# erthward/geonomics

Measured on AMD Instinct MI355X. Metric: individual-timesteps/sec, higher is better.
Workload: dtype u64

## Files before the change

geonomics_amd/_native.py:

```python
import ctypes as C
import os

import numpy as np

_HERE = os.path.dirname(os.path.abspath(__file__))
LIB_PATH = os.environ.get('GNX_LIB') or os.path.join(_HERE, 'libgnxhip.so')

DIST = {'lognormal': 0, 'wald': 1, 'levy': 2}
MATE_UNIFORM, MATE_NEAREST, MATE_INVERSE = 0, 1, 2
SURF_NONE, SURF_MIXTURE, SURF_UNIMODAL = 0, 1, 2
(F_X, F_Y, F_AGE, F_SEX, F_ID, F_E, F_Z, F_FIT, F_GROW, F_GENO) = range(10)
(R_N, R_NPAIRS, R_K, R_D, R_COUNTS) = range(5)
KERNELS = ['move', 'sort', 'permute', 'find_mates', 'pairs', 'offspring',
           'crossover', 'phenotype', 'density', 'death', 'compact', 'crossover_tail']

EXPORTS = [
    'gnx_create', 'gnx_destroy', 'gnx_last_error', 'gnx_words_per_hom', 'gnx_blocks_per_hom',
    'gnx_set_stream', 'gnx_synchronize', 'gnx_upload_rasters',
    'gnx_upload_layer', 'gnx_set_species_params', 'gnx_upload_population',
    'gnx_init_population', 'gnx_set_recomb_paths', 'gnx_set_trait',
    'gnx_set_dominance', 'gnx_set_deleterious', 'gnx_upload_genomes',
    'gnx_assign_genomes', 'gnx_set_z', 'gnx_age', 'gnx_move',
    'gnx_pop_dynamics', 'gnx_pop_dynamics_mate', 'gnx_pop_dynamics_die',
    'gnx_set_z_range', 'gnx_step', 'gnx_counts', 'gnx_step_index',
# ... 371 lines not shown
        cnt = np.zeros(64, np.int64)
        self._chk(self.lib.gnx_tile2_vt_counts(self.h, _ptr(cnt, C.c_int64)))
        return cnt

    def tile2_vt_bases(self, bases):
        b = _arr(bases, np.int64)
        assert b.size == 64
        self._chk(self.lib.gnx_tile2_vt_bases(self.h, _ptr(b, C.c_int64)))

    def step_begin(self, burn):
        self._chk(self.lib.gnx_step_begin(self.h, int(bool(burn))))

    def step_mid(self, burn, with_selection):
        self._chk(self.lib.gnx_step_mid(self.h, int(bool(burn)), int(bool(with_selection))))

    def step_end(self, burn):
        self._chk(self.lib.gnx_step_end(self.h, int(bool(burn))))

    def counts(self):
        n, b, d = C.c_int64(), C.c_int64(), C.c_int64()
        self._chk(self.lib.gnx_counts(self.h, C.byref(n), C.byref(b), C.byref(d)))
        return n.value, b.value, d.value

    def totals(self):
        out = np.zeros(6, np.int64)
        self._chk(self.lib.gnx_totals(self.h, _ptr(out, C.c_int64)))
        return dict(zip(('steps', 'ind_steps', 'births', 'deaths', 'xo_births', 'dd_steps'),
                        (int(v) for v in out)))

    def reset_totals(self):
        self._chk(self.lib.gnx_reset_totals(self.h))

    PATH_COUNTS = ('lazy_mortalities', 'xo_launch_p2', 'xo_flush', 'jobs_lanes_256',
                   'jobs_lanes_512', 'sort_hist_gather', 'gc_with_pending_xo', 'make_dense')

    def path_counts(self):
        out = np.zeros(len(self.PATH_COUNTS), np.int64)
        n = self.lib.gnx_path_counts(self.h, _ptr(out, C.c_int64), len(out))
        assert n == len(out), 'gnx_path_counts: the library has %d counters' % n
        return dict(zip(self.PATH_COUNTS, (int(v) for v in out)))

    def reset_path_counts(self):
        self._chk(self.lib.gnx_reset_path_counts(self.h))

    @property
    def N(self):
        return self.counts()[0]

    @property
    def step_index(self):
        return self.lib.gnx_step_index(self.h)

    @step_index.setter
    def step_index(self, v):
        self._chk(self.lib.gnx_set_step_index(self.h, C.c_int64(int(v))))

    def synchronize(self):
        self._chk(self.lib.gnx_synchronize(self.h))

    def set_defer_crossover(self, on):
        self._chk(self.lib.gnx_set_defer_crossover(self.h, int(bool(on))))

    def set_crossover_overlap(self, mode):
        self._chk(self.lib.gnx_set_crossover_overlap(self.h, int(mode)))

    def debug_halves(self):
        out = np.zeros(6, np.int64)
# ... 1054 lines not shown
```

geonomics_amd/csrc/gnx_api.hip:

```cpp
#include <cmath>
#include <cstdarg>
#include <algorithm>
#include <atomic>
#include <chrono>
#include "gnx_internal.h"
#include "gnx_rng.h"
#include "gnx_compact.h"

static thread_local char g_err[1024] = "";

void gnx_set_error(const char* fmt, ...) {
  va_list ap;
  va_start(ap, fmt);
  vsnprintf(g_err, sizeof(g_err), fmt, ap);
  va_end(ap);
}

extern "C" const char* gnx_last_error(void) { return g_err; }

extern "C" int gnx_words_per_hom(int32_t L) {
  int w = (L + 63) / 64;
  return ((w + 15) / 16) * 16;
}

// ... 289 lines not shown
      }
      h->row_spread = want;
    }
    GNXCHK(dalloc(&h->free_rows, (size_t)h->cfg.cap_rows));
    const size_t halves = (size_t)h->cfg.cap_rows * h->row_spread * 2 * h->NB;
    GNXCHK(dalloc(&h->hmap, halves));
    GNXCHK(dalloc(&h->half_mark, halves));
    GNXCHK(dalloc(&h->half_free, (size_t)h->cfg.cap_rows * 2 * h->NB));
    GNXCHK(dalloc(&h->half_top, 1));
    HIPCHK(hipMalloc(&h->xo_plan, (size_t)cap * 40));
    GNXCHK(dalloc(&h->gc_cnt, (size_t)h->cfg.cap_rows * 2 * h->NB / GNX_CB + 2));
    GNXCHK(dalloc(&h->gc_off, (size_t)h->cfg.cap_rows * 2 * h->NB / GNX_CB + 2));
    HIPCHK(hipMemset(h->half_mark, 0, halves));
    HIPCHK(hipMalloc((void**)&h->xo_jobs_acc, 2 * sizeof(unsigned long long)));
    HIPCHK(hipMemset(h->xo_jobs_acc, 0, 2 * sizeof(unsigned long long)));
    HIPCHK(hipMemset(h->hmap, 0xff, halves * sizeof(int32_t)));
    HIPCHK(hipMemset(h->half_top, 0, sizeof(int32_t)));
    h->alias_xo = gnx_env_int("GNX_XO_ALIAS", 1) != 0;
  }
  for (int k = 0; k < 2; ++k) {
    GNXCHK(dalloc(&h->key[k], cap));
    GNXCHK(dalloc(&h->perm[k], cap));
  }
  GNXCHK(dalloc(&h->mate, cap));
  for (int k = 0; k < 2; ++k) {
    GNXCHK(dalloc(&h->ord[k], cap));
    GNXCHK(dalloc(&h->keyk[k], cap));
    GNXCHK(dalloc(&h->valk[k], cap));
  }
  GNXCHK(dalloc(&h->newslot, cap));
  GNXCHK(dalloc(&h->fill_cnt, 4));
  HIPCHK(hipEventCreateWithFlags(&h->ev_fill, gnx_order_event_flags()));
  HIPCHK(hipEventCreateWithFlags(&h->ev_alive, gnx_order_event_flags()));
  HIPCHK(hipEventCreateWithFlags(&h->ev_perm_rest, gnx_order_event_flags()));
  {
    const size_t nb = std::max(gnx_os_scratch_bytes((size_t)cap, 24),
                               gnx_os_words_used64((size_t)cap, 64) * sizeof(unsigned int)) + 16;
    HIPCHK(hipMalloc(&h->os_scratch, nb));
    HIPCHK(hipMemset(h->os_scratch, 0, nb));
  }
  GNXCHK(dalloc(&h->os_ktmp, cap));
  GNXCHK(dalloc(&h->os_vtmp, cap));
  GNXCHK(dalloc(&h->cell32, cap));
  GNXCHK(dalloc(&h->ord_cnt, cap / GNX_CB + 2));
  GNXCHK(dalloc(&h->ord_off, cap / GNX_CB + 2));
  HIPCHK(hipEventCreateWithFlags(&h->ev_ord, gnx_order_event_flags()));
  HIPCHK(hipStreamCreate(&h->stream3));
  HIPCHK(hipEventCreateWithFlags(&h->ev_compact, gnx_order_event_flags()));
  h->ord_mode = gnx_env_int("GNX_ORD_SORT", 1) != 0;
  GNXCHK(dalloc(&h->tag, cap));
  HIPCHK(hipMalloc(&h->cand, (size_t)cap * 16));
  GNXCHK(dalloc(&h->flag, cap + 1));
  GNXCHK(dalloc(&h->flag2, cap + 1));
  GNXCHK(dalloc(&h->scan, cap + 1));
  GNXCHK(dalloc(&h->pairs, cap * 2));
  GNXCHK(dalloc(&h->nbirths, cap + 1));
  GNXCHK(dalloc(&h->boff, cap + 1));
  GNXCHK(dalloc(&h->off_pair, cap));
  GNXCHK(dalloc(&h->off_parent, cap * 2));
  GNXCHK(dalloc(&h->off_keys, cap * 2));
  GNXCHK(dalloc(&h->off_start, cap * 2));
  GNXCHK(dalloc(&h->keep_in, cap));
  GNXCHK(dalloc(&h->inj_a, cap * GNX_DISP_ATTEMPTS));
  GNXCHK(dalloc(&h->inj_b, cap * GNX_DISP_ATTEMPTS));
  GNXCHK(dalloc(&h->mid_x, cap));
  GNXCHK(dalloc(&h->mid_y, cap));
// ... 89 lines not shown
                  h->delet_loci, h->delet_s, h->cell_start, h->tag, h->cand, h->sort64_tmp, h->key64[0], h->key64[1], h->pairs2,
                  h->pair_goff, h->st_rec, h->st_z, h->st_geno, h->st_slots, h->req_pid, h->req_k, h->req_key, h->req_start, h->req_px, h->req_py,
                  h->req_count, h->sort_tmp, h->scan_tmp, h->mate,
                  h->flag, h->flag2, h->scan, h->pairs, h->nbirths, h->boff, h->off_pair,
                  h->off_parent, h->off_keys, h->off_start, h->keep_in, h->inj_a, h->inj_b,
                  h->mid_x, h->mid_y, h->p_death, h->d_cell, h->dead_in, h->nmax_bits, h->red,
                  h->sel_loci, h->path_sel, h->lat.areas, h->lat.cprime, h->spl_N.c, h->spl_P.c, h->bin_partials, h->nodes,
                  h->K_over, h->blk_cnt, h->blk_off, h->cnt_dev, h->tickets, h->nmax2, h->fb[0], h->gp_rec, h->gp_z, h->gp_slots, h->tile_counts, h->rq_sorted, h->rq_k, h->gam_out, h->gam_slot, h->chk,
                  h->lin_tab, h->lin_bt};
  for (void* p : ptrs) (void)hipFree(p);
  for (int t = 0; t < GNX_MAX_TRAITS; ++t) {
    (void)hipFree(h->traits[t].loci);
    (void)hipFree(h->traits[t].alpha);
    (void)hipFree(h->traits[t].phi_rast);
  }
  (void)hipHostFree(h->h_pin);
  if (h->h_route_pin) (void)hipHostFree(h->h_route_pin);
  (void)hipFree(h->gh_rec);
  (void)hipFree(h->route_cnt);
  if (h->h_stage) (void)hipHostFree(h->h_stage);
  for (int k = 0; k < GNX_K_COUNT; ++k) timers_resolve(h, k);
  for (hipEvent_t e : h->ev_free) (void)hipEventDestroy(e);
  if (h->own_stream) (void)hipStreamDestroy(h->stream);
  if (h->stream2) (void)hipStreamDestroy(h->stream2);
  h->stream2 = nullptr;
  if (h->stream3) {
    (void)hipStreamSynchronize(h->stream3);
    (void)hipStreamDestroy(h->stream3);
  }
  if (h->ev_ord) (void)hipEventDestroy(h->ev_ord);
  if (h->ev_compact) (void)hipEventDestroy(h->ev_compact);
  if (h->ev_fill) (void)hipEventDestroy(h->ev_fill);
  if (h->ev_alive) (void)hipEventDestroy(h->ev_alive);
  if (h->ev_perm_rest) (void)hipEventDestroy(h->ev_perm_rest);
  if (h->ev_pairs) (void)hipEventDestroy(h->ev_pairs);
  if (h->ev_latP) (void)hipEventDestroy(h->ev_latP);
  if (h->ev_perm) (void)hipEventDestroy(h->ev_perm);
  if (h->ev_binsN) (void)hipEventDestroy(h->ev_binsN);
  delete h;
}

extern "C" int gnx_set_stream(gnx_state* h, void* hip_stream) {
  GNXCHK(gnx_xo_join(h));
  HIPCHK(hipStreamSynchronize(h->stream));
  if (h->stream2) HIPCHK(hipStreamSynchronize(h->stream2));
  if (h->own_stream) (void)hipStreamDestroy(h->stream);
  if (h->stream2) (void)hipStreamDestroy(h->stream2);
  h->stream2 = nullptr;
  h->stream = (hipStream_t)hip_stream;
  h->own_stream = false;
  return 0;
}

extern "C" int gnx_synchronize(gnx_state* h) {
  GNXCHK(gnx_xo_launch_pending(h));
  if (h->stream3) HIPCHK(hipStreamSynchronize(h->stream3));
  HIPCHK(hipStreamSynchronize(h->stream));
  if (h->stream2) HIPCHK(hipStreamSynchronize(h->stream2));
  return 0;
}

extern "C" int gnx_upload_rasters(gnx_state* h, const float* rasts) {
  size_t n = (size_t)h->cfg.n_layers * h->cfg.W * h->cfg.H;
  HIPCHK(hipMemcpyAsync(h->rast, rasts, n * sizeof(float), hipMemcpyHostToDevice, h->stream));
  HIPCHK(hipStreamSynchronize(h->stream));
  return 0;
// ... 497 lines not shown
  return 0;
}

extern "C" int gnx_pop_dynamics(gnx_state* h, int32_t burn, int32_t with_selection) {
  GNXCHK(gnx_pop_dynamics_mate(h, burn));
  return gnx_pop_dynamics_die(h, burn, with_selection);
}

struct GnxStepTimer {
  std::chrono::steady_clock::time_point t0 = std::chrono::steady_clock::now();
  bool count;
  explicit GnxStepTimer(bool c) : count(c) {}
  ~GnxStepTimer() {
    if (gnx_host_times()) {
      g_host_step_s += std::chrono::duration<double>(std::chrono::steady_clock::now() - t0).count();
      if (count) ++g_host_steps;
    }
  }
};

extern "C" int gnx_step_begin(gnx_state* h, int32_t burn) {
  GNXCHK(need_params(h));
  GNXCHK(check_recomb_ready(h, burn != 0));
  GnxStepTimer timer(true);
  if (h->mort_wait || h->pairs_wait) {
    gnx_set_error("gnx_step_begin: the previous step of this handle was not finished (gnx_step_end)");
    return 1;
  }
  h->tot[0] += 1;
  h->tot[1] += h->N - h->n_ghost;
  h->last_xo_births = 0;
  h->step_burn = burn != 0;
  h->tile2_mode = false;
  if (h->sp.move) {
    h->move_writes_keys = h->sp.mating_radius >= 0;
    int rc = gnx_l_move(h, true, nullptr, nullptr, nullptr, nullptr, true);
    h->move_writes_keys = false;
    GNXCHK(rc);
  } else {
    GNXCHK(gnx_l_age(h));
  }
  GNXCHK(gnx_l_sort_by_cell(h, true));
  int rc_pairs = gnx_l_find_pairs_enqueue(h, nullptr, true);
  GNXCHK(gnx_wait_permute_rest(h));
  return rc_pairs;
}

extern "C" int gnx_step_mid(gnx_state* h, int32_t burn, int32_t with_selection) {
  GnxStepTimer timer(false);
  int64_t P = 0, B = 0;
  GNXCHK(gnx_l_find_pairs_finish(h, &P));
  if (P > 0 && !h->spl_P.valid)
    GNXCHK(gnx_l_density(h, P, h->mid_x, h->mid_y, &h->spl_P, nullptr));
  GNXCHK(gnx_l_mate(h, burn != 0, false, 0, &B));
  h->last_births = B;
  GNXCHK(gnx_l_density_N(h));
  GNXCHK(gnx_l_death_probs(h, with_selection != 0 && !burn));
  return gnx_l_mortality_enqueue(h, nullptr);
}

extern "C" int gnx_step_end(gnx_state* h, int32_t burn) {
  GnxStepTimer timer(false);
  int64_t D = 0;
  GNXCHK(gnx_l_mortality_finish(h, &D));
  h->last_deaths = D;
  h->step += 1;
  h->tot[2] += h->last_births;
// ... 527 lines not shown
```

geonomics_amd/csrc/gnx_dd.hip:

```cpp
#include <atomic>
#include <chrono>
#include <map>
#include <string>
#include "gnx_internal.h"

bool gnx_fused_bins(const gnx_state* h);

namespace {
using GraphMap = std::map<uint32_t, hipGraphExec_t>;

struct DDExtra {
  GraphMap graphs;
  hipStream_t cap = nullptr;
  bool capturing = false;
  uint64_t epoch = 0;
};

DDExtra* extra(gnx_state* h) {
  if (!h->dd_graph[0]) h->dd_graph[0] = new DDExtra();
  return (DDExtra*)h->dd_graph[0];
}

bool dd_debug() { return gnx_env_int("GNX_DD_DEBUG", 0) != 0; }
}
// ... 393 lines not shown
  for (int k = 0; k < n; ++k) {
    bool ok = false;
    hs[k]->dd_hist.clear();
    hs[k]->dd_hist_closed = false;
    const int64_t n0 = hs[k]->N - hs[k]->n_ghost;
    GNXCHK(walk_prepare(hs[k], &left[k], burn != 0, with_selection != 0, &ok));
    if (left[k] < T) {
      hs[k]->dd_hist.push_back(n0);
      hs[k]->dd_hist.push_back(hs[k]->last_births);
      hs[k]->dd_hist.push_back(hs[k]->last_deaths);
    }
    dd[k] = ok && left[k] > 0;
    if (dd[k]) {
      const int rc_enter = dd_enter(hs[k]);
      if (rc_enter) {
        dd[k] = 0;
        for (int q = 0; q < k; ++q)
          if (dd[q]) (void)gnx_dd_leave(hs[q]);
        return rc_enter;
      }
    }
  }
  int rc = 0;
  for (bool any = true; any && !rc;) {
    any = false;
    for (int k = 0; k < n && !rc; ++k) {
      if (left[k] <= 0) continue;
      int64_t taken = 1;
      if (dd[k]) {
        rc = dd_some(hs[k], burn != 0, with_selection != 0, left[k], &taken);
      } else {
        const int64_t n0 = hs[k]->N - hs[k]->n_ghost;
        hs[k]->eager_move = left[k] > 1;
        rc = gnx_step(hs[k], burn, with_selection);
        hs[k]->eager_move = false;
        if (!rc) {
          hs[k]->dd_hist.push_back(n0);
          hs[k]->dd_hist.push_back(hs[k]->last_births);
          hs[k]->dd_hist.push_back(hs[k]->last_deaths);
        }
      }
      left[k] -= taken;
      any = any || left[k] > 0;
    }
  }
  for (int k = 0; k < n; ++k)
    if (dd[k]) {
      const int r2 = gnx_dd_leave(hs[k]);
      if (!rc) rc = r2;
    }
  {
    const std::string first_err = rc ? std::string(gnx_last_error()) : std::string();
    for (int k = 0; k < n; ++k) {
      const int r3 = gnx_l_make_dense(hs[k]);
      if (!rc) rc = r3;
    }
    if (!first_err.empty()) gnx_set_error("%s", first_err.c_str());
  }
  if (gnx_host_times()) {
    g_host_step_s += std::chrono::duration<double>(std::chrono::steady_clock::now() - t0).count();
    g_host_steps += T * n;
  }
  return rc;
}

extern "C" int64_t gnx_walk_history(gnx_state* h, int64_t max_steps, int64_t* n_start,
                                    int64_t* births, int64_t* deaths) {
  const int64_t total = (int64_t)h->dd_hist.size() / 3;
// ... 10 lines not shown
```

geonomics_amd/csrc/gnx_internal.h:

```cpp
#pragma once
#include <cstring>
#include <cstdint>
#include <cstdio>
#include <cstdlib>
#include <string>
#include <vector>
#include <utility>
#include <hip/hip_runtime.h>
#include "../../include/gnx_hip.h"
#include "gnx_half.h"

#define GNX_MAX_TRAITS 16
#define GNX_MAX_LAYERS 16
#define GNX_DISP_ATTEMPTS 8
#define GNX_SPARSE_MAX_BP 24

void gnx_set_error(const char* fmt, ...);

static inline int gnx_env_int(const char* name, int dflt) {
  const char* v = getenv(name);
  return v ? atoi(v) : dflt;
}
static inline int64_t gnx_dd_max_cap() {
  static const int64_t v = getenv("GNX_DD_MAX_CAP") ? atoll(getenv("GNX_DD_MAX_CAP")) : 600000;
// ... 180 lines not shown
  unsigned long long todo = __ballot(dest >= 0);
  const int lane = threadIdx.x & 63;
  int idx = -1;
  while (todo) {
    const int leader = __ffsll((long long)todo) - 1;
    const int d = __shfl(dest, leader);
    const unsigned long long same = __ballot(dest == d);
    int base = 0;
    if (lane == leader) base = atomicAdd(&counts[d], (int)__popcll(same));
    base = __shfl(base, leader);
    if (dest == d) idx = base + (int)__popcll(same & ((1ull << lane) - 1ull));
    todo &= ~same;
  }
  return idx;
}
__device__ __forceinline__ int gnx_route_dest(const RouteGeo& g, int k, int orow, int oc, int cx, int cy) {
  if (k == 4) return (orow * g.C + oc) != g.me ? orow * g.C + oc : -1;
  const int rr = orow + k / 3 - 1, cc = oc + k % 3 - 1;
  if (rr >= 0 && rr < g.R && cc >= 0 && cc < g.C && cx >= g.cx0[cc] && cx <= g.cx1[cc] &&
      cy >= g.cy0[rr] && cy <= g.cy1[rr])
    return rr * g.C + cc;
  return -1;
}
#endif
enum {
  GNX_PC_LAZY_MORT = 0,
  GNX_PC_XO_P2,
  GNX_PC_XO_FLUSH,
  GNX_PC_JOBS_256,
  GNX_PC_JOBS_512,
  GNX_PC_SORT_GATHER,
  GNX_PC_GC_PENDING_XO,
  GNX_PC_MAKE_DENSE,
  GNX_PC_COUNT
};

struct gnx_state {
  gnx_config cfg{};
  gnx_species_params sp{};
  bool have_sp = false;
  hipStream_t stream = nullptr;
  hipStream_t stream2 = nullptr;
  bool xo_pending = false;
  bool own_stream = false;
  int W64 = 0;
  int64_t N = 0;
  int64_t max_id = -1;
  int64_t step = 0;
  int64_t last_births = 0, last_deaths = 0;
  int64_t tot[6]{};
  int64_t pc[GNX_PC_COUNT]{};
  int64_t n_ghost = 0;

  GnxSoA soa[2]{};
  int cur = 0;

  uint64_t* G = nullptr;
  int row_spread = 1;
  int32_t* free_rows = nullptr;
  int64_t n_free = 0;
  int32_t* hmap = nullptr;
  uint8_t* half_mark = nullptr;
  int32_t* half_free = nullptr;
  int32_t* half_top = nullptr;
  int64_t half_free_est = 0;
  int64_t gc_runs = 0;
// ... 216 lines not shown
  bool perm_rest_pending = false;
  GnxSoA perm_rest_a{}, perm_rest_b{};
  int64_t perm_rest_N = 0;
  hipEvent_t ev_perm_rest = nullptr;
  bool fb_pending = false;
  const float *fbp_x = nullptr, *fbp_y = nullptr;
  int64_t fbp_N = 0;
  hipEvent_t ev_alive = nullptr;
  int32_t* fill_cnt = nullptr;
  hipEvent_t ev_fill = nullptr;
  int64_t fill_guess = 0;
  uint32_t* cell32 = nullptr;
  uint32_t* keyk[2]{};
  int32_t* valk[2]{};
  void* os_scratch = nullptr;
  uint32_t* os_ktmp = nullptr;
  int32_t* os_vtmp = nullptr;
  int32_t* ord_cnt = nullptr;
  int32_t* ord_off = nullptr;
  hipEvent_t ev_ord = nullptr;
  bool ord_inflight = false;
  bool keys_ordmode = false;
  bool keys_fresh = false;
  bool hist_fresh = false;
  bool holes = false;
  int64_t holes_N = 0;
  RouteGeo* route_geo_dev = nullptr;
  uint64_t route_geo_epoch = 0;
  bool move_counts_routes = false;
  bool move_counted_routes = false;
  bool tile_lazy_ok = false;
  int64_t holes_flagged = 0;
  bool eager_move = false;
  bool move_writes_keys = false;
  int n_bin_blocks = 0;
  double* nodes = nullptr;
  double* K_over = nullptr;
  unsigned long long* nmax_bits = nullptr;
  double* p_death = nullptr;
  double* d_cell = nullptr;
  uint8_t* dead_in = nullptr;
  int32_t* counts_rast[2]{};
  int counts_cur = 0;
  bool counts_init = false;
  double* red = nullptr;

  int32_t* blk_cnt = nullptr;
  int32_t* blk_off = nullptr;
  int blk_stride = 0;
  int32_t* cnt_dev = nullptr;
  unsigned int* tickets = nullptr;

  int64_t* h_pin = nullptr;
  int64_t* h_pin_dev = nullptr;
  int64_t pin_seq = 0;
  void* h_stage = nullptr;
  size_t h_stage_bytes = 0;

  void* tile_comm = nullptr;
  GnxDD* dd = nullptr;
  GnxDDRec* dd_ring = nullptr;
  GnxDDRec* dd_ring_dev = nullptr;
  bool dd_active = false;
  int64_t dd_seq = 0;
  int64_t dd_seen = 0;
  int64_t dd_half_est = 0;
// ... 16 lines not shown
  hipEvent_t ev_open = nullptr;
  std::vector<hipEvent_t> ev_free;
  std::vector<std::pair<hipEvent_t, hipEvent_t>> ev_pending[GNX_K_COUNT];
};

GnxTraitTab gnx_trait_tab(const gnx_state* h);

static inline GnxHalves gnx_halves(const gnx_state* h) {
  return GnxHalves{h->hmap, h->half_free, h->half_top, h->NB, h->BW > 0 ? h->BW : h->W64 / h->NB};
}
int gnx_half_reserve(gnx_state* h, int64_t blocks);
int gnx_gc(gnx_state* h);
static inline const int32_t* gnx_alias_bp(const gnx_state* h) {
  return (h->alias_xo && h->sparse_paths) ? h->bp_off : nullptr;
}
static inline const int32_t* gnx_alias_loci(const gnx_state* h) {
  return (h->alias_xo && h->sparse_paths) ? h->bp_loci : nullptr;
}

int gnx_publish(gnx_state* h, int slot, const int32_t* a, const int32_t* b = nullptr,
                const int32_t* c = nullptr, const int32_t* d = nullptr);

void gnx_time_begin(gnx_state* h, int kernel = -1);
void gnx_time_end(gnx_state* h, int kernel, double bytes);

int gnx_h2d(gnx_state* h, void* dst, const void* src, size_t bytes);
int gnx_d2h(gnx_state* h, void* dst, const void* src, size_t bytes);

int gnx_l_init_population(gnx_state* h, int64_t N);
int gnx_l_gather_e(gnx_state* h, int64_t first, int64_t n);
int gnx_l_age(gnx_state* h);
int gnx_l_move(gnx_state* h, bool inc_age, const float* inj_theta, const float* inj_dist,
               float* out_theta, float* out_dist, bool apply);
int gnx_l_sort_by_cell(gnx_state* h, bool split_rest = false);
int gnx_wait_permute_rest(gnx_state* h);
int gnx_permute_rest_launch(gnx_state* h);
int gnx_l_find_pairs(gnx_state* h, const uint8_t* d_keep, int64_t* n_pairs_out,
                     bool with_density = false);
int gnx_l_find_pairs_enqueue(gnx_state* h, const uint8_t* d_keep, bool with_density);
int gnx_l_find_pairs_finish(gnx_state* h, int64_t* n_pairs_out);
int gnx_l_births(gnx_state* h, int64_t* births_out);
int gnx_l_pair_cls(gnx_state* h, int64_t P, bool local);
int gnx_vt_buffers(gnx_state* h);
int gnx_l_mate(gnx_state* h, bool burn, bool inject, int64_t B_inject, int64_t* births_out,
               int64_t id_base = -1, bool tiled = false);
int gnx_l_dispersal_inject(gnx_state* h, int64_t B, int A, const float* d_mx, const float* d_my,
                           const float* d_theta, const float* d_dist, float* d_ox, float* d_oy,
                           int32_t* d_used);
int gnx_l_crossover_all(gnx_state* h, int64_t first_slot, int64_t B);
int gnx_l_crossover_requests(gnx_state* h, int64_t first_slot, int64_t n_req);
int gnx_l_crossover_pending(gnx_state* h, int64_t first_slot, int64_t B);
int gnx_l_crossover_survivors(gnx_state* h, int64_t first_slot, int64_t B, const int32_t* d_alive,
                              const int32_t* d_scan);
int gnx_xo_join(gnx_state* h);
int gnx_xo_flush_deferred(gnx_state* h);
int gnx_xo_launch_pending(gnx_state* h, int site = GNX_PC_XO_FLUSH);
int gnx_xo_wait_inflight(gnx_state* h);
int gnx_xo_prepare_jobs(gnx_state* h, int32_t** zero);
int gnx_xo_wait_wide(gnx_state* h);
double gnx_xo_bytes_per_birth(const gnx_state* h);
int gnx_l_rebuild_sel(gnx_state* h);
int gnx_l_path_sel(gnx_state* h);
int gnx_l_tb_from_rows(gnx_state* h, int64_t first, int64_t n, const int32_t* d_list,
                       const int64_t* d_slots, bool join = true);
int gnx_l_newborn_tb(gnx_state* h, int64_t first_slot, int64_t B);
int gnx_l_phenotype(gnx_state* h, int64_t first_slot, int64_t n, const int32_t* d_list = nullptr);
// ... 163 lines not shown
```

geonomics_amd/csrc/gnx_kernels_demog.hip:

```cpp
#include "gnx_internal.h"
#include <chrono>
#include "gnx_rng.h"
#include "gnx_compact.h"
#include "gnx_half.h"
#include "gnx_xo.h"

#define BIN_BLOCKS 512

__global__ void __launch_bounds__(256)
k_bins(int64_t n, const int32_t* n_dev, const float* x, const float* y, const uint8_t* ghost,
       double inv_hww, int nbx, int nby, int32_t* partials, GnxSetWords sw) {
  extern __shared__ int32_t lds_hist[];
  if (sw.dst && blockIdx.x == 0 && threadIdx.x < 4) sw.dst[threadIdx.x] = sw.v[threadIdx.x];
  if (n_dev) n = *n_dev;
  const int nb = nbx * nby;
  for (int k = threadIdx.x; k < nb; k += blockDim.x) lds_hist[k] = 0;
  __syncthreads();
  const int64_t stride = (int64_t)gridDim.x * blockDim.x;
  for (int64_t i = (int64_t)blockIdx.x * blockDim.x + threadIdx.x; i < n; i += stride) {
    if (ghost && ghost[i]) continue;
    int hx = min(nbx - 1, (int)floor((double)x[i] * inv_hww));
    int hy = min(nby - 1, (int)floor((double)y[i] * inv_hww));
    atomicAdd(&lds_hist[hy * nbx + hx], 1);
  }
// ... 1609 lines not shown
  *deaths_out = 0;
  GNXCHK(gnx_l_mortality_enqueue(h, d_dead_inject));
  return gnx_l_mortality_finish(h, deaths_out);
}

int gnx_l_mortality_enqueue(gnx_state* h, const uint8_t* d_dead_inject) {
  int64_t N = h->N;
  h->mort_wait = false;
  gnx_bins_adults_drop(h);
  if (N == 0) return 0;
  const gnx_config& c = h->cfg;
  GnxSoA a = h->soa[h->cur], b = h->soa[h->cur ^ 1];
  const int nb = (int)((N + GNX_CB - 1) / GNX_CB);
  const bool xo = h->xo_deferred;
  const int64_t xo_first = h->xo_first, xo_B = xo ? h->xo_B : 0;
  const bool ord_keep = h->ord_mode && h->ord_valid && !h->tiled;
  int32_t* zero_jobs = nullptr;
  if (xo) {
    GNXCHK(gnx_xo_prepare_jobs(h, &zero_jobs));
    GNXCHK(gnx_half_reserve(h, 2 * (int64_t)h->NB * xo_B));
  }
  gnx_time_begin(h);
  hipLaunchKernelGGL(k_alive, dim3(nb), dim3(256), 0, h->stream, N, h->p_death, d_dead_inject,
                     a.id, a.ghost, a.grow, h->step, c.seed, h->flag, h->flag2, h->blk_cnt,
                     h->blk_stride, xo ? xo_first : (int64_t)-1, zero_jobs, (const GnxDD*)nullptr,
                     GnxScanOut{});
  const bool fill = h->compact_fill && h->stream3 != nullptr && d_dead_inject == nullptr;
  const bool side_scan = fill && xo && xo_B > 0 && jobs_fused_ok(h);
  const bool lazy_common = fill && h->sp.move && h->sp.mating_radius >= 0;
  const bool lazy_tile = lazy_common && gnx_env_int("GNX_TILE_LAZY", 0) != 0 && h->tile_lazy_ok &&
                         h->tile2_mode && h->tile_R * h->tile_C > 1 && !ord_keep;
  const bool lazy = lazy_tile || (lazy_common && h->eager_move && ord_keep && h->key_bits <= 24 &&
                                  h->n_ghost == 0 && !h->tile2_mode);
  if (side_scan) {
    HIPCHK(hipEventRecord(h->ev_alive, h->stream));
    HIPCHK(hipStreamWaitEvent(h->stream3, h->ev_alive, 0));
    GNXCHK(gnx_block_scan(h, 3, N, h->blk_cnt, h->blk_off, h->cnt_dev, h->h_pin_dev, 0, h->stream3));
    gnx_time_end(h, GNX_K_COMPACT, 0.0);
    HIPCHK(hipEventRecord(h->ev_counts, h->stream3));
  } else {
    GNXCHK(gnx_block_scan(h, 3, N, h->blk_cnt, h->blk_off, h->cnt_dev, h->h_pin_dev));
    gnx_time_end(h, GNX_K_COMPACT, 0.0);
    HIPCHK(hipEventRecord(h->ev_counts, h->stream));
  }
  h->jobs_self_scan = side_scan;
  int has_rows = (h->genomes_assigned && c.L > 0) ? 1 : 0;
  if (fill && !lazy) {
    if (!side_scan) HIPCHK(hipStreamWaitEvent(h->stream3, h->ev_counts, 0));
    hipLaunchKernelGGL(k_fill_lists, dim3(nb), dim3(256), 0, h->stream3, N, h->flag, h->flag2,
                       h->blk_off, h->blk_stride, h->cnt_dev, a.grow, has_rows,
                       (int32_t*)h->os_ktmp, (int32_t*)h->os_ktmp + c.cap_inds / 2,
                       (int32_t*)h->os_vtmp, ord_keep ? h->newslot : nullptr, h->fill_cnt,
                       (const GnxDD*)nullptr, GnxOrdF{});
    HIPCHK(hipEventRecord(h->ev_fill, h->stream3));
  }
  if (xo) {
    h->xo_deferred = false;
    GNXCHK(gnx_l_crossover_survivors(h, xo_first, xo_B, h->flag, h->blk_off));
    h->jobs_self_scan = false;
    if (h->xo_sort_waits && h->xo_wait_at == 2) GNXCHK(gnx_xo_wait_inflight(h));
  }
  if (ord_keep && h->ord_inflight) HIPCHK(hipStreamWaitEvent(h->stream, h->ev_ord, 0));
  gnx_time_begin(h);
  const double rec_bytes = 34.0 + 4.0 * c.n_layers + 4.0 * c.n_traits + 16.0 * h->TW;
  if (lazy) {
    if (has_rows) {
      if (side_scan) HIPCHK(hipStreamWaitEvent(h->stream, h->ev_counts, 0));
      hipLaunchKernelGGL(k_dead_rows, dim3(nb), dim3(256), 0, h->stream, N,
                         (const int32_t*)h->flag2, (const int32_t*)(h->blk_off + h->blk_stride),
                         a.grow, (const int32_t*)h->cnt_dev, xo ? 1 : 0,
                         h->free_rows, h->n_free);
    }
    gnx_time_end(h, GNX_K_COMPACT, (double)N * 8.0);
    h->holes = true;
    h->holes_N = N;
    h->holes_flagged = N;
    ++h->pc[GNX_PC_LAZY_MORT];
  } else if (fill) {
    HIPCHK(hipStreamWaitEvent(h->stream, h->ev_fill, 0));
    const int64_t guess = std::max<int64_t>(h->fill_guess * 2, 4096);
    const int fb_ = (int)std::min<int64_t>(gnx_grid(std::min<int64_t>(guess, N), 256), 8192);
    hipLaunchKernelGGL(k_fill, dim3(fb_), dim3(256), 0, h->stream, c.cap_inds, h->fill_cnt,
                       (const int32_t*)h->os_ktmp, (const int32_t*)h->os_ktmp + c.cap_inds / 2,
                       h->cnt_dev, a, c.n_layers, c.n_traits, a.tb ? 2 * h->TW : 0,
                       (const int32_t*)h->os_vtmp, h->free_rows, h->n_free, has_rows, xo ? 1 : 0,
                       ord_keep ? h->newslot : nullptr, (const GnxDD*)nullptr);
    gnx_time_end(h, GNX_K_COMPACT, (double)N * 16.0 + (double)h->fill_guess * (16.0 + 2.0 * rec_bytes));
  } else {
    hipLaunchKernelGGL(k_compact, dim3(nb), dim3(256), 0, h->stream, N, c.cap_inds, h->flag,
                       h->flag2, h->blk_off, h->blk_stride, h->cnt_dev, a, b, c.n_layers, c.n_traits,
                       a.tb ? 2 * h->TW : 0, h->free_rows, h->n_free, has_rows, xo ? 1 : 0,
                       ord_keep ? h->newslot : nullptr);
    gnx_time_end(h, GNX_K_COMPACT, (double)N * (24.0 + 2.0 * rec_bytes));
  }
  if (ord_keep) {
    HIPCHK(hipEventRecord(h->ev_compact, h->stream));
    HIPCHK(hipStreamWaitEvent(h->stream3, h->ev_compact, 0));
    if (h->ord_inflight) h->ord_inflight = false;
    GnxScanOut So{h->ord_off, nullptr, nullptr, 0, nullptr, h->tickets + 2, h->blk_stride};
    hipLaunchKernelGGL(k_ord_flags, dim3(nb), dim3(256), 0, h->stream3, N, h->ord_n,
                       h->ord[h->ord_cur], h->newslot, h->ord_cnt, So, (const GnxDD*)nullptr,
                       lazy ? (const int32_t*)h->flag : (const int32_t*)nullptr);
    hipLaunchKernelGGL(k_ord_write, dim3(nb), dim3(256), 0, h->stream3, N, h->ord_n,
                       h->ord[h->ord_cur], h->newslot, h->ord_off, h->ord[h->ord_cur ^ 1],
                       (const GnxDD*)nullptr, GnxDDEnd{}, 0,
                       lazy ? (const int32_t*)h->flag : (const int32_t*)nullptr);
    h->ord_covers_xo = false;
    if (h->xo_sort_waits && !h->xo_last_split && h->xo_ready_buf < 0) {
      for (int k = 0; k < 2; ++k)
        if (h->xo_inflight[k]) HIPCHK(hipStreamWaitEvent(h->stream3, h->ev_xo_done[k], 0));
      h->ord_covers_xo = true;
    }
    HIPCHK(hipEventRecord(h->ev_ord, h->stream3));
    h->ord_inflight = true;
    h->ord_cur ^= 1;
  } else {
    h->ord_valid = false;
  }
  HIPCHK(hipGetLastError());
  h->mort_wait = true;
  h->mort_xo = xo;
  h->mort_fill = fill;
  h->mort_ord_keep = ord_keep;
  h->mort_has_rows = has_rows;
  h->mort_N = N;
  return 0;
}

int gnx_l_mortality_finish(gnx_state* h, int64_t* deaths_out) {
  *deaths_out = 0;
  if (!h->mort_wait) return 0;
  h->mort_wait = false;
  const bool xo = h->mort_xo, fill = h->mort_fill, ord_keep = h->mort_ord_keep;
  const int has_rows = h->mort_has_rows;
  const int64_t N = h->mort_N;
  {
    const bool ht = gnx_host_times();
    const auto t0 = std::chrono::steady_clock::now();
    HIPCHK(hipEventSynchronize(h->ev_counts));
    if (ht) g_host_wait_s += std::chrono::duration<double>(std::chrono::steady_clock::now() - t0).count();
    gnx_host_mark(2);
  }
  const int64_t survivors = h->h_pin[0];
  const int64_t rows_freed = h->h_pin[1];
  if (xo) {
    const int64_t S = h->h_pin[2];
    h->n_free -= S;
    h->last_xo_births = S;
  }
  if (has_rows) h->n_free += rows_freed;
  *deaths_out = N - h->n_ghost - survivors;
  h->fill_guess = N - survivors;
  h->N = survivors;
  h->n_ghost = 0;
  if (survivors == 0) h->holes = false;
  if (!fill) h->cur ^= 1;
  if (ord_keep) h->ord_n = survivors;
  return 0;
}


int gnx_dd_l_density_N(gnx_state* h, int par, hipStream_t st) {
  const GnxLattice& L = h->lat;
  const int64_t nn = (int64_t)L.Jx * L.Jy;
  const size_t lat_doubles = (size_t)4 * nn + std::max(L.Jx, L.Jy) + 1;
  const int nmax_R = gnx_nmax_rows_fit(L.Jx, lat_doubles);
  const size_t lds_bytes = (lat_doubles + gnx_nmax_lds_doubles(L.Jx, nmax_R)) * sizeof(double);
  hipLaunchKernelGGL(k_lattice_nmax, dim3(std::max(1, std::min(h->cfg.H, GNX_LATN_BLOCKS)) + 1), dim3(256),
                     lds_bytes, st, L.Jx, L.Jy, L.nbx, (const int32_t*)h->fb[par], L.areas, L.hww,
                     L.cprime, h->spl_N.c, h->cfg.W, h->cfg.H, h->nmax2 + par, h->fb[par ^ 1],
                     h->nmax2 + (par ^ 1), h->fb[2], h->spl_P.c, GnxPubWords{}, nmax_R, gnx_nmax_scan_min());
  HIPCHK(hipGetLastError());
  return 0;
}

int gnx_dd_l_death_probs(gnx_state* h, bool with_selection, int par, hipStream_t st) {
  h->spl_N.valid = h->spl_P.valid = true;
  SplineC SN = make_splinec(h, h->spl_N), SP = make_splinec(h, h->spl_P);
  DeathP Q = make_deathp(h, with_selection);
  Q.dd = h->dd;
  hipLaunchKernelGGL(k_death_probs, dim3(gnx_grid(h->cfg.cap_inds, 256)), dim3(256), 0, st, Q,
                     make_demp(h), SN, SP, h->soa[h->cur], h->rast, gnx_trait_tab(h), h->delet_s,
                     (const unsigned long long*)(h->nmax2 + par), h->p_death, h->d_cell);
  HIPCHK(hipGetLastError());
  return 0;
}

int gnx_dd_l_alive(gnx_state* h, bool xo, int buf, hipStream_t st) {
// ... 125 lines not shown
```

geonomics_amd/csrc/gnx_kernels_pop.hip:

```cpp
#include "gnx_internal.h"
#include "gnx_rng.h"
#include "gnx_compact.h"
#include "gnx_tb.h"
#include "gnx_bins.h"

static int gnx_id_bits(const gnx_state* h) {
  int b = 1;
  while (b < 40 && (h->max_id >> b) != 0) ++b;
  return b;
}
static bool gnx_ord_sort(const gnx_state* h) {
  return h->ord_mode && h->ord_valid && !h->tiled;
}

__device__ __forceinline__ int wave_min_i(int v) {
#pragma unroll
  for (int m = 32; m >= 1; m >>= 1) v = min(v, __shfl_xor(v, m));
  return v;
}
__device__ __forceinline__ int wave_max_i(int v) {
#pragma unroll
  for (int m = 32; m >= 1; m >>= 1) v = max(v, __shfl_xor(v, m));
  return v;
}
// ... 358 lines not shown
      }
      for (int k = 0; k < 9; ++k) {
        const int dest = act[u] ? gnx_route_dest(g, k, orow, oc, hx, hy) : -1;
        if (__ballot(dest >= 0) == 0ull) continue;
        (void)gnx_route_append(P.rcnt + (k == 4 ? 0 : T), dest);
      }
    }
  }
  if (P.hist) {
    __syncthreads();
    for (int q = threadIdx.x; q < P.hist_places << P.hist_rb; q += 256) {
      const uint32_t v = mhist[q];
      if (v) atomicAdd(&P.hist[q], v);
    }
  }
}

int gnx_os_hist_discard(gnx_state* h, hipStream_t st) {
  if (!h->hist_fresh) return 0;
  h->hist_fresh = false;
  HIPCHK(hipMemsetAsync(h->os_scratch, 0, GNX_MOVE_HIST_WORDS * sizeof(uint32_t), st ? st : h->stream));
  return 0;
}

static bool gnx_move_hist(const gnx_state* h, int* places, int* rb) {
  gnx_os_digits(h->key_bits, places, rb);
  return h->os_scratch != nullptr && (*places << *rb) <= GNX_MOVE_HIST_WORDS;
}

int gnx_l_move(gnx_state* h, bool inc_age, const float* inj_theta, const float* inj_dist,
               float* out_theta, float* out_dist, bool apply) {
  const bool ddm = h->dd_active;
  if (!ddm && h->N == 0) return 0;
  if (apply) {
    h->fb_adults = false;
    h->fb_pending = false;
  }
  const gnx_config& c = h->cfg;
  const gnx_species_params& sp = h->sp;
  MoveP P;
  P.dd = ddm ? h->dd : nullptr;
  P.alive = nullptr;
  P.N = h->N;
  const bool holes = h->holes && apply && !ddm && !inj_theta;
  if (h->holes && !holes) {
    gnx_set_error("internal: a movement other than the step's own over an uncompacted population");
    return 1;
  }
  if (holes) {
    P.alive = h->flag;
    P.N = h->holes_N;
  }
  P.cap = c.cap_inds;
  P.W = c.W;
  P.H = c.H;
  P.n_layers = c.n_layers;
  P.xmax = (float)(c.W - 0.001);
  P.ymax = (float)(c.H - 0.001);
  P.rrx = (float)sp.res_ratio[0];
  P.rry = (float)sp.res_ratio[1];
  P.distr = sp.move_distr;
  P.p1 = (float)sp.move_p1;
  P.p2 = (float)sp.move_p2;
  P.mu = (float)sp.dir_mu;
  P.kappa = (float)sp.dir_kappa;
  P.surf = sp.move_surf;
// ... 11 lines not shown
  P.inv_cs = h->inv_cs;
  P.ncx = h->ncx;
  P.ncy = h->ncy;
  P.idbits = gnx_id_bits(h);
  GNXCHK(gnx_os_hist_discard(h));
  P.hist = nullptr;
  P.hist_rb = P.hist_places = 0;
  if (ordm && !ddm && gnx_move_hist(h, &P.hist_places, &P.hist_rb)) {
    P.hist = (uint32_t*)h->os_scratch;
    h->hist_fresh = true;
  }
  P.rg = nullptr;
  P.rcnt = nullptr;
  if (h->move_counts_routes && apply && !ddm && !inj_theta && h->route_geo_dev && h->route_cnt) {
    P.rg = h->route_geo_dev;
    P.rcnt = h->route_cnt;
    h->move_counted_routes = true;
  }
  h->keys_fresh = with_keys;
  if (with_keys) h->keys_ordmode = ordm;
  constexpr int GNX_MOVE_TILE_FLOATS = 2 * 2048;
  P.tile_floats = sp.move_surf != GNX_SURF_NONE ? GNX_MOVE_TILE_FLOATS : 0;
  gnx_time_begin(h);
  const int64_t n_grid = ddm ? (int64_t)c.cap_inds : (holes ? h->holes_N : h->N);
  hipLaunchKernelGGL(k_move<2>, dim3(gnx_grid(n_grid, 512)), dim3(256),
                     (size_t)P.tile_floats * sizeof(float), h->stream, P,
                     h->soa[h->cur], h->rast, inj_theta, inj_dist, out_theta, out_dist);
  gnx_time_end(h, GNX_K_MOVE,
               (double)h->N * (32.0 + 8.0 * c.n_layers + (sp.move_surf ? 36.0 : 0.0)));
  HIPCHK(hipGetLastError());
  return 0;
}

__device__ __forceinline__ int gnx_cell_of(float x, float y, double inv_cs, int ncx, int ncy) {
  int cx = min(ncx - 1, (int)((double)x * inv_cs));
  int cy = min(ncy - 1, (int)((double)y * inv_cs));
  return cy * ncx + cx;
}

__global__ void k_keys(int64_t N, const float* x, const float* y, const int64_t* id,
                       double inv_cs, int ncx, int ncy, int idbits, uint64_t* key, int32_t* idx) {
  int64_t i = (int64_t)blockIdx.x * blockDim.x + threadIdx.x;
  if (i >= N) return;
  key[i] = ((uint64_t)gnx_cell_of(x[i], y[i], inv_cs, ncx, ncy) << idbits) | (uint64_t)id[i];
  idx[i] = (int32_t)i;
}

__global__ void k_keys_evict(int64_t N, const float* x, const float* y, const int64_t* id,
                             const uint8_t* ghost, float x0, float x1, float y0, float y1,
                             double inv_cs, int ncx, int ncy, int idbits, uint64_t* key,
                             int32_t* idx, const int32_t* __restrict__ alive, int64_t n_flagged) {
  int64_t i = (int64_t)blockIdx.x * blockDim.x + threadIdx.x;
  if (i >= N) return;
  const float xi = x[i], yi = y[i];
  const bool dead = alive != nullptr && i < n_flagged && (alive[i] & 1) == 0;
  const bool out = !ghost[i] && (xi < x0 || xi >= x1 || yi < y0 || yi >= y1);
  const uint64_t cell = dead ? (uint64_t)(ncx * ncy) + 1ull
                             : (out ? (uint64_t)(ncx * ncy) : (uint64_t)gnx_cell_of(xi, yi, inv_cs, ncx, ncy));
  key[i] = (cell << idbits) | (uint64_t)id[i];
  idx[i] = (int32_t)i;
}

__global__ void k_free_tail(int64_t N, int64_t n, const int32_t* grow, int32_t* free_rows,
                            int64_t n_free) {
  int64_t k = (int64_t)blockIdx.x * blockDim.x + threadIdx.x;
  if (k < n) free_rows[n_free + k] = grow[N + k];
// ... 126 lines not shown
  GNXCHK(gnx_permute_rest_launch(h));
  if (h->perm_rest_inflight) {
    HIPCHK(hipStreamWaitEvent(h->stream, h->ev_perm_rest, 0));
    h->perm_rest_inflight = false;
  }
  return 0;
}

__global__ void k_gather_ord(int64_t N, int64_t cap, const int32_t* __restrict__ ord, GnxSoA a,
                             GnxSoA b, int n_layers, int n_traits, int tbw,
                             int32_t* __restrict__ ord_new) {
  const int64_t i = (int64_t)blockIdx.x * blockDim.x + threadIdx.x;
  if (i >= N) return;
  const int64_t j = ord[i];
  const GnxRec r = gnx_rec_load(a, j, cap, n_layers, n_traits, tbw);
  gnx_rec_store(b, i, cap, n_layers, n_traits, tbw, r);
  gnx_rec_rest(a, j, b, i, cap, n_layers, n_traits, tbw);
  ord_new[i] = (int32_t)i;
}

int gnx_l_make_dense(gnx_state* h) {
  if (!h->holes) return 0;
  if (h->tile2_mode || h->mort_wait || h->pairs_wait || !h->ord_valid || h->ord_n != h->N) {
    gnx_set_error("internal: an uncompacted population that cannot be gathered (tile %d, step "
                  "open %d, index %d with %lld of %lld)", (int)h->tile2_mode,
                  (int)(h->mort_wait || h->pairs_wait), (int)h->ord_valid, (long long)h->ord_n,
                  (long long)h->N);
    return 1;
  }
  const int64_t N = h->N;
  gnx_bins_adults_drop(h);
  GNXCHK(gnx_wait_permute_rest(h));
  GNXCHK(gnx_xo_flush_deferred(h));
  GNXCHK(gnx_os_hist_discard(h));
  h->keys_fresh = false;
  if (h->ord_inflight) {
    HIPCHK(hipStreamWaitEvent(h->stream, h->ev_ord, 0));
    h->ord_inflight = false;
  }
  const gnx_config& c = h->cfg;
  GnxSoA a = h->soa[h->cur], b = h->soa[h->cur ^ 1];
  hipLaunchKernelGGL(k_gather_ord, dim3(gnx_grid(N, 256)), dim3(256), 0, h->stream, N, c.cap_inds,
                     (const int32_t*)h->ord[h->ord_cur], a, b, c.n_layers, c.n_traits,
                     a.tb ? 2 * h->TW : 0, h->ord[h->ord_cur ^ 1]);
  HIPCHK(hipGetLastError());
  h->cur ^= 1;
  h->ord_cur ^= 1;
  h->holes = false;
  h->holes_N = 0;
  h->holes_flagged = 0;
  ++h->pc[GNX_PC_MAKE_DENSE];
  return 0;
}

int gnx_l_sort_by_cell(gnx_state* h, bool split_rest) {
  int64_t N = h->N;
  gnx_bins_adults_drop(h);
  GNXCHK(gnx_wait_permute_rest(h));
  if (N == 0) {
    h->holes = false;
    return 0;
  }
  GNXCHK(gnx_xo_flush_deferred(h));
  const bool xo_covered = h->xo_sort_waits && h->ord_covers_xo && h->ord_inflight && h->tile_evict == 0 &&
                          (h->keys_fresh ? h->keys_ordmode : gnx_ord_sort(h));
  if (xo_covered) {
    for (int k = 0; k < 2; ++k) h->xo_inflight[k] = h->xo_wide_inflight[k] = false;
    h->ord_covers_xo = false;
  } else if (h->xo_sort_waits) {
    GNXCHK(gnx_xo_wait_wide(h));
  }
  const gnx_config& c = h->cfg;
  GnxSoA a = h->soa[h->cur], b = h->soa[h->cur ^ 1];
  const int idbits = gnx_id_bits(h);
  const bool alone = h->xo_sort_waits || !h->xo_running;
  const bool tile_holes = h->holes && h->tile2_mode;
  const int64_t n_sort = tile_holes ? h->holes_N : N;
  const bool ordm = (h->tile_evict > 0 || tile_holes) ? false
                                                      : (h->keys_fresh ? h->keys_ordmode : gnx_ord_sort(h));
  if (h->holes && !tile_holes && !(ordm && h->keys_fresh)) {
    gnx_set_error("internal: the cell sort of an uncompacted population needs the id-ordered index "
                  "and the movement's keys");
    return 1;
  }
  h->holes = false;
  gnx_time_begin(h);
  int64_t wipe_words = 0;
  if (ordm) {
    if (!h->keys_fresh)
      hipLaunchKernelGGL(k_cells, dim3(gnx_grid(N, 256)), dim3(256), 0, h->stream, N, a.x, a.y,
                         h->inv_cs, h->ncx, h->ncy, h->cell32);
    if (h->ord_inflight) {
      HIPCHK(hipStreamWaitEvent(h->stream, h->ev_ord, 0));
      h->ord_inflight = false;
// ... 1521 lines not shown
```

Before: 2.444 billion.

## Run next step's movement ahead on a side stream during compaction

When a lazy ord-keep compaction runs inside a multi-step density-dependent loop, the next step's movement kernel is launched early on stream2, gated on the alive-flag event, and joined at the start of the next step. The ord index rebuild moves onto the main stream in that path, and several join points (sort, make_dense, zero survivors) are added to keep state consistent. The goal is to overlap movement with compaction and the later stages of the current step. The cost is more cross-stream state juggling: the step counter, stream and holes fields are temporarily rewritten, which risks ordering bugs, and the path only applies when several gating conditions hold.

```diff
diff --git a/geonomics_amd/_native.py b/geonomics_amd/_native.py
--- a/geonomics_amd/_native.py
+++ b/geonomics_amd/_native.py
@@ -427,7 +427,8 @@
         self._chk(self.lib.gnx_reset_totals(self.h))
 
     PATH_COUNTS = ('lazy_mortalities', 'xo_launch_p2', 'xo_flush', 'jobs_lanes_256',
-                   'jobs_lanes_512', 'sort_hist_gather', 'gc_with_pending_xo', 'make_dense')
+                   'jobs_lanes_512', 'sort_hist_gather', 'gc_with_pending_xo', 'make_dense',
+                   'moves_ahead')
 
     def path_counts(self):
         out = np.zeros(len(self.PATH_COUNTS), np.int64)
diff --git a/geonomics_amd/csrc/gnx_api.hip b/geonomics_amd/csrc/gnx_api.hip
--- a/geonomics_amd/csrc/gnx_api.hip
+++ b/geonomics_amd/csrc/gnx_api.hip
@@ -345,6 +345,7 @@
   GNXCHK(dalloc(&h->fill_cnt, 4));
   HIPCHK(hipEventCreateWithFlags(&h->ev_fill, gnx_order_event_flags()));
   HIPCHK(hipEventCreateWithFlags(&h->ev_alive, gnx_order_event_flags()));
+  HIPCHK(hipEventCreateWithFlags(&h->ev_moved, gnx_order_event_flags()));
   HIPCHK(hipEventCreateWithFlags(&h->ev_perm_rest, gnx_order_event_flags()));
   {
     const size_t nb = std::max(gnx_os_scratch_bytes((size_t)cap, 24),
@@ -500,6 +501,7 @@
   if (h->ev_compact) (void)hipEventDestroy(h->ev_compact);
   if (h->ev_fill) (void)hipEventDestroy(h->ev_fill);
   if (h->ev_alive) (void)hipEventDestroy(h->ev_alive);
+  if (h->ev_moved) (void)hipEventDestroy(h->ev_moved);
   if (h->ev_perm_rest) (void)hipEventDestroy(h->ev_perm_rest);
   if (h->ev_pairs) (void)hipEventDestroy(h->ev_pairs);
   if (h->ev_latP) (void)hipEventDestroy(h->ev_latP);
@@ -1063,7 +1065,9 @@
   h->last_xo_births = 0;
   h->step_burn = burn != 0;
   h->tile2_mode = false;
-  if (h->sp.move) {
+  if (h->moved_ahead) {
+    GNXCHK(gnx_move_ahead_join(h));
+  } else if (h->sp.move) {
     h->move_writes_keys = h->sp.mating_radius >= 0;
     int rc = gnx_l_move(h, true, nullptr, nullptr, nullptr, nullptr, true);
     h->move_writes_keys = false;
diff --git a/geonomics_amd/csrc/gnx_dd.hip b/geonomics_amd/csrc/gnx_dd.hip
--- a/geonomics_amd/csrc/gnx_dd.hip
+++ b/geonomics_amd/csrc/gnx_dd.hip
@@ -449,8 +449,9 @@
       } else {
         const int64_t n0 = hs[k]->N - hs[k]->n_ghost;
         hs[k]->eager_move = left[k] > 1;
+        hs[k]->move_ahead_ok = n == 1 && left[k] > 1;
         rc = gnx_step(hs[k], burn, with_selection);
-        hs[k]->eager_move = false;
+        hs[k]->eager_move = hs[k]->move_ahead_ok = false;
         if (!rc) {
           hs[k]->dd_hist.push_back(n0);
           hs[k]->dd_hist.push_back(hs[k]->last_births);
diff --git a/geonomics_amd/csrc/gnx_internal.h b/geonomics_amd/csrc/gnx_internal.h
--- a/geonomics_amd/csrc/gnx_internal.h
+++ b/geonomics_amd/csrc/gnx_internal.h
@@ -236,6 +236,7 @@
   GNX_PC_SORT_GATHER,
   GNX_PC_GC_PENDING_XO,
   GNX_PC_MAKE_DENSE,
+  GNX_PC_MOVE_AHEAD,
   GNX_PC_COUNT
 };
 
@@ -518,6 +519,9 @@
   bool tile_lazy_ok = false;
   int64_t holes_flagged = 0;
   bool eager_move = false;
+  bool move_ahead_ok = false;
+  bool moved_ahead = false;
+  hipEvent_t ev_moved = nullptr;
   bool move_writes_keys = false;
   int n_bin_blocks = 0;
   double* nodes = nullptr;
@@ -600,6 +604,8 @@
 int gnx_l_age(gnx_state* h);
 int gnx_l_move(gnx_state* h, bool inc_age, const float* inj_theta, const float* inj_dist,
                float* out_theta, float* out_dist, bool apply);
+int gnx_l_move_ahead(gnx_state* h, int64_t N);
+int gnx_move_ahead_join(gnx_state* h);
 int gnx_l_sort_by_cell(gnx_state* h, bool split_rest = false);
 int gnx_wait_permute_rest(gnx_state* h);
 int gnx_permute_rest_launch(gnx_state* h);
diff --git a/geonomics_amd/csrc/gnx_kernels_demog.hip b/geonomics_amd/csrc/gnx_kernels_demog.hip
--- a/geonomics_amd/csrc/gnx_kernels_demog.hip
+++ b/geonomics_amd/csrc/gnx_kernels_demog.hip
@@ -1665,8 +1665,11 @@
                          h->tile2_mode && h->tile_R * h->tile_C > 1 && !ord_keep;
   const bool lazy = lazy_tile || (lazy_common && h->eager_move && ord_keep && h->key_bits <= 24 &&
                                   h->n_ghost == 0 && !h->tile2_mode);
+  const bool move_ahead = lazy && ord_keep && h->move_ahead_ok && h->stream2 != nullptr &&
+                          h->xo_launch_late;
+  const bool lazy_ord = lazy && ord_keep;
+  if (side_scan || lazy_ord) HIPCHK(hipEventRecord(h->ev_alive, h->stream));
   if (side_scan) {
-    HIPCHK(hipEventRecord(h->ev_alive, h->stream));
     HIPCHK(hipStreamWaitEvent(h->stream3, h->ev_alive, 0));
     GNXCHK(gnx_block_scan(h, 3, N, h->blk_cnt, h->blk_off, h->cnt_dev, h->h_pin_dev, 0, h->stream3));
     gnx_time_end(h, GNX_K_COMPACT, 0.0);
@@ -1693,7 +1696,24 @@
     h->jobs_self_scan = false;
     if (h->xo_sort_waits && h->xo_wait_at == 2) GNXCHK(gnx_xo_wait_inflight(h));
   }
+  if (move_ahead) GNXCHK(gnx_l_move_ahead(h, N));
   if (ord_keep && h->ord_inflight) HIPCHK(hipStreamWaitEvent(h->stream, h->ev_ord, 0));
+  auto ord_launch = [&](hipStream_t os) {
+    GnxScanOut So{h->ord_off, nullptr, nullptr, 0, nullptr, h->tickets + 2, h->blk_stride};
+    hipLaunchKernelGGL(k_ord_flags, dim3(nb), dim3(256), 0, os, N, h->ord_n,
+                       h->ord[h->ord_cur], h->newslot, h->ord_cnt, So, (const GnxDD*)nullptr,
+                       lazy ? (const int32_t*)h->flag : (const int32_t*)nullptr);
+    hipLaunchKernelGGL(k_ord_write, dim3(nb), dim3(256), 0, os, N, h->ord_n,
+                       h->ord[h->ord_cur], h->newslot, h->ord_off, h->ord[h->ord_cur ^ 1],
+                       (const GnxDD*)nullptr, GnxDDEnd{}, 0,
+                       lazy ? (const int32_t*)h->flag : (const int32_t*)nullptr);
+  };
+  if (move_ahead) {
+    ord_launch(h->stream);
+    h->ord_inflight = false;
+    h->ord_covers_xo = false;
+    h->ord_cur ^= 1;
+  }
   gnx_time_begin(h);
   const double rec_bytes = 34.0 + 4.0 * c.n_layers + 4.0 * c.n_traits + 16.0 * h->TW;
   if (lazy) {
@@ -1726,18 +1746,16 @@
                        ord_keep ? h->newslot : nullptr);
     gnx_time_end(h, GNX_K_COMPACT, (double)N * (24.0 + 2.0 * rec_bytes));
   }
-  if (ord_keep) {
-    HIPCHK(hipEventRecord(h->ev_compact, h->stream));
-    HIPCHK(hipStreamWaitEvent(h->stream3, h->ev_compact, 0));
+  if (move_ahead) {
+  } else if (ord_keep) {
+    if (!lazy_ord) {
+      HIPCHK(hipEventRecord(h->ev_compact, h->stream));
+      HIPCHK(hipStreamWaitEvent(h->stream3, h->ev_compact, 0));
+    } else if (!side_scan) {
+      HIPCHK(hipStreamWaitEvent(h->stream3, h->ev_alive, 0));
+    }
     if (h->ord_inflight) h->ord_inflight = false;
-    GnxScanOut So{h->ord_off, nullptr, nullptr, 0, nullptr, h->tickets + 2, h->blk_stride};
-    hipLaunchKernelGGL(k_ord_flags, dim3(nb), dim3(256), 0, h->stream3, N, h->ord_n,
-                       h->ord[h->ord_cur], h->newslot, h->ord_cnt, So, (const GnxDD*)nullptr,
-                       lazy ? (const int32_t*)h->flag : (const int32_t*)nullptr);
-    hipLaunchKernelGGL(k_ord_write, dim3(nb), dim3(256), 0, h->stream3, N, h->ord_n,
-                       h->ord[h->ord_cur], h->newslot, h->ord_off, h->ord[h->ord_cur ^ 1],
-                       (const GnxDD*)nullptr, GnxDDEnd{}, 0,
-                       lazy ? (const int32_t*)h->flag : (const int32_t*)nullptr);
+    ord_launch(h->stream3);
     h->ord_covers_xo = false;
     if (h->xo_sort_waits && !h->xo_last_split && h->xo_ready_buf < 0) {
       for (int k = 0; k < 2; ++k)
@@ -1786,7 +1804,14 @@
   h->fill_guess = N - survivors;
   h->N = survivors;
   h->n_ghost = 0;
-  if (survivors == 0) h->holes = false;
+  if (survivors == 0) {
+    h->holes = false;
+    if (h->moved_ahead) {
+      GNXCHK(gnx_move_ahead_join(h));
+      GNXCHK(gnx_os_hist_discard(h));
+      h->keys_fresh = false;
+    }
+  }
   if (!fill) h->cur ^= 1;
   if (ord_keep) h->ord_n = survivors;
   return 0;
diff --git a/geonomics_amd/csrc/gnx_kernels_pop.hip b/geonomics_amd/csrc/gnx_kernels_pop.hip
--- a/geonomics_amd/csrc/gnx_kernels_pop.hip
+++ b/geonomics_amd/csrc/gnx_kernels_pop.hip
@@ -414,6 +414,10 @@
                float* out_theta, float* out_dist, bool apply) {
   const bool ddm = h->dd_active;
   if (!ddm && h->N == 0) return 0;
+  if (h->moved_ahead) {
+    gnx_set_error("internal: a movement while the next step's own is already in flight");
+    return 1;
+  }
   if (apply) {
     h->fb_adults = false;
     h->fb_pending = false;
@@ -491,6 +495,33 @@
   return 0;
 }
 
+int gnx_l_move_ahead(gnx_state* h, int64_t N) {
+  HIPCHK(hipStreamWaitEvent(h->stream2, h->ev_alive, 0));
+  h->holes = true;
+  h->holes_N = N;
+  h->holes_flagged = N;
+  hipStream_t main = h->stream;
+  h->stream = h->stream2;
+  h->step += 1;
+  h->move_writes_keys = true;
+  const int rc = gnx_l_move(h, true, nullptr, nullptr, nullptr, nullptr, true);
+  h->move_writes_keys = false;
+  h->step -= 1;
+  h->stream = main;
+  GNXCHK(rc);
+  HIPCHK(hipEventRecord(h->ev_moved, h->stream2));
+  h->moved_ahead = true;
+  ++h->pc[GNX_PC_MOVE_AHEAD];
+  return 0;
+}
+
+int gnx_move_ahead_join(gnx_state* h) {
+  if (!h->moved_ahead) return 0;
+  h->moved_ahead = false;
+  HIPCHK(hipStreamWaitEvent(h->stream, h->ev_moved, 0));
+  return 0;
+}
+
 __device__ __forceinline__ int gnx_cell_of(float x, float y, double inv_cs, int ncx, int ncy) {
   int cx = min(ncx - 1, (int)((double)x * inv_cs));
   int cy = min(ncy - 1, (int)((double)y * inv_cs));
@@ -683,6 +714,7 @@
   gnx_bins_adults_drop(h);
   GNXCHK(gnx_wait_permute_rest(h));
   GNXCHK(gnx_xo_flush_deferred(h));
+  GNXCHK(gnx_move_ahead_join(h));
   GNXCHK(gnx_os_hist_discard(h));
   h->keys_fresh = false;
   if (h->ord_inflight) {
@@ -710,7 +742,7 @@
   GNXCHK(gnx_wait_permute_rest(h));
   if (N == 0) {
     h->holes = false;
-    return 0;
+    return gnx_move_ahead_join(h);
   }
   GNXCHK(gnx_xo_flush_deferred(h));
   const bool xo_covered = h->xo_sort_waits && h->ord_covers_xo && h->ord_inflight && h->tile_evict == 0 &&
```

Result: faster. 2.533 billion, median of 6 (+3.7%).
